# aliftffd/ViT-vs-Raw-IQ

Measured on AMD Instinct MI355X. Metric: IQ frames/sec training (fwd+loss+bwd+clip+AdamW), higher is better.
Workload: dtype bf16; 1 GPU; ViT-Tiny/16 224x224 C=1 19cls (BASELINE configs[1]); config_id=B, per_gpu_batch=256, global_batch=256, parallelism=dp1, hipgraph=True

## Files before the change

### vit-vs-raw-iq_amd/csrc/attention.hip

```cpp
#include <stdlib.h>

#include "common.h"
#include "iqvit.h"
#include "prof.h"

namespace {

constexpr int ATT_THREADS = 512;
constexpr int ATT_WAVES = ATT_THREADS / 64;
constexpr float LOG2E = 1.4426950408889634f;
constexpr float LN2 = 0.6931471805599453f;
constexpr float NEG_BIG = -1.0e30f;

__device__ __forceinline__ float fast_exp2(float x) { return __builtin_amdgcn_exp2f(x); }

template <int DH> struct AttCfg {
  static constexpr int LD = (DH == 16) ? 16 : DH + 16;
  static constexpr int KS = (DH + 31) / 32;
  static constexpr int DT = DH / 16;
  static constexpr int CPR = DH / 8;
};

typedef __attribute__((address_space(3))) s16x4 lds_s16x4;

__device__ __forceinline__ bf16x8 tr_frag(const bf16* tile, int ld, int r0, int c0, int lane) {
  const int i16 = lane & 15, g = lane >> 4;
  const bf16* a = tile + (r0 + 4 * g + (i16 >> 2)) * ld + c0 + 4 * (i16 & 3);
  s16x4 lo = __builtin_amdgcn_ds_read_tr16_b64_v4i16((lds_s16x4*)(a));
  s16x4 hi = __builtin_amdgcn_ds_read_tr16_b64_v4i16((lds_s16x4*)(a + 16 * ld));
  s16x8 v = {lo[0], lo[1], lo[2], lo[3], hi[0], hi[1], hi[2], hi[3]};
  return __builtin_bit_cast(bf16x8, v);
}

template <int DH>
__device__ __forceinline__ bf16x8 row_frag_lds(const bf16* tile, int row, int s, int lane) {
  const int d0 = s * 32 + 8 * (lane >> 4);
  bf16x8 v = {};
  if (DH >= 32 || d0 < DH) v = *reinterpret_cast<const bf16x8*>(tile + row * AttCfg<DH>::LD + d0);
  return v;
}
template <int DH>
__device__ __forceinline__ bf16x8 row_frag_gmem(const bf16* base, long ldg, int row, int nrows, int s, int lane) {
  const int d0 = s * 32 + 8 * (lane >> 4);
  bf16x8 v = {};
  if (row < nrows && (DH >= 32 || d0 < DH)) v = *reinterpret_cast<const bf16x8*>(base + (long)row * ldg + d0);
  return v;
}

template <int DH>
__device__ __forceinline__ void stage_rows(bf16* img, const bf16* base, long ldg, int r_begin, int nrows_pad, int S,
                                           int tid) {
  constexpr int CPR = AttCfg<DH>::CPR, LD = AttCfg<DH>::LD;
  for (int id = tid; id < nrows_pad * CPR; id += ATT_THREADS) {
    const int r = id / CPR, c = id % CPR;
    bf16x8 v = {};
    if (r_begin + r < S) v = *reinterpret_cast<const bf16x8*>(base + (long)(r_begin + r) * ldg + c * 8);
    *reinterpret_cast<bf16x8*>(img + r * LD + c * 8) = v;
  }
}

template <int DH, int UN>
__device__ __forceinline__ void stage_pair(bf16* imgA, const bf16* baseA, long ldgA, bf16* imgB, const bf16* baseB, long ldgB,
                                           int r_begin, int nrows_pad, int S, int tid) {
  constexpr int CPR = AttCfg<DH>::CPR, LD = AttCfg<DH>::LD;
  const int total = nrows_pad * CPR;
  for (int base = 0; base < total; base += UN * ATT_THREADS) {
    bf16x8 va[UN], vb[UN];
#pragma unroll
    for (int j = 0; j < UN; ++j) {
      const int id = min(base + j * ATT_THREADS + tid, total - 1);
      const int r = min(r_begin + id / CPR, S - 1), c = id % CPR;
      va[j] = *reinterpret_cast<const bf16x8*>(baseA + (long)r * ldgA + c * 8);
      vb[j] = *reinterpret_cast<const bf16x8*>(baseB + (long)r * ldgB + c * 8);
    }
#pragma unroll
    for (int j = 0; j < UN; ++j) {
      const int id = base + j * ATT_THREADS + tid;
      const int r = id / CPR, c = id % CPR;
      if (id < total) {
        const bool live = r_begin + r < S;
        *reinterpret_cast<bf16x8*>(imgA + r * LD + c * 8) = live ? va[j] : bf16x8{};
        *reinterpret_cast<bf16x8*>(imgB + r * LD + c * 8) = live ? vb[j] : bf16x8{};
      }
    }
  }
}

__device__ __forceinline__ bf16x8 pack_b(const f32x4& lo, const f32x4& hi) {
  bf16x8 v;
#pragma unroll
  for (int r = 0; r < 4; ++r) { v[r] = (bf16)lo[r]; v[4 + r] = (bf16)hi[r]; }
  return v;
}

__device__ __forceinline__ float group4_max(float v) {
  v = fmaxf(v, __shfl_xor(v, 16, 64));
  return fmaxf(v, __shfl_xor(v, 32, 64));
}
__device__ __forceinline__ float group4_sum(float v) {
  v += __shfl_xor(v, 16, 64);
  return v + __shfl_xor(v, 32, 64);
}

template <int DH, bool MASKED>
__global__ __launch_bounds__(ATT_THREADS) void attn_fwd_kernel(const bf16* __restrict__ qkv, bf16* __restrict__ out,
                                                               float* __restrict__ lse, const uint8_t* __restrict__ mask,
                                                               long mask_hstride, int S, int H, int kchunk,
                                                               float scale_log2, float masked_raw) {
  using C = AttCfg<DH>;
  extern __shared__ __attribute__((aligned(16))) unsigned char smem[];
  bf16* Ks = reinterpret_cast<bf16*>(smem);
  bf16* Vs = Ks + kchunk * C::LD;
  const int tid = threadIdx.x, lane = tid & 63, wave = tid >> 6, g = lane >> 4, c16 = lane & 15;
  const int b = blockIdx.x / H, h = blockIdx.x % H;
  const int D = H * DH;
  const long ldg = 3L * D;
  const bf16* qb = qkv + (long)b * S * ldg + h * DH;
  const bf16* kb_ = qb + D;
  const bf16* vb_ = qb + 2 * D;
  const uint8_t* mk = MASKED ? mask + (long)b * (mask_hstride ? (long)H * S * S : (long)S * S) + h * mask_hstride : nullptr;
  const int qtiles = (S + 31) / 32, npass = (qtiles + ATT_WAVES - 1) / ATT_WAVES, nstage = (S + kchunk - 1) / kchunk;

  if (nstage == 1) {
    stage_pair<DH, 4>(Ks, kb_, ldg, Vs, vb_, ldg, 0, min(kchunk, ((S + 31) / 32) * 32), S, tid);
    __syncthreads();
  }
  for (int pass = 0; pass < npass; ++pass) {
    const int qt = pass * ATT_WAVES + wave;
    const bool active = qt < qtiles;
    bf16x8 qf[2][C::KS];
    f32x4 o[2][C::DT];
    float m[2], lsum[2];
#pragma unroll
    for (int u = 0; u < 2; ++u) {
      m[u] = NEG_BIG; lsum[u] = 0.f;
#pragma unroll
      for (int s = 0; s < C::KS; ++s) qf[u][s] = row_frag_gmem<DH>(qb, ldg, qt * 32 + u * 16 + c16, active ? S : 0, s, lane);
#pragma unroll
      for (int dt = 0; dt < C::DT; ++dt) o[u][dt] = f32x4{0.f, 0.f, 0.f, 0.f};
    }
    for (int st = 0; st < nstage; ++st) {
      const int k0 = st * kchunk;
      const int krows = min(kchunk, ((S - k0 + 31) / 32) * 32);
      if (nstage > 1) {
        __syncthreads();
        stage_pair<DH, 2>(Ks, kb_, ldg, Vs, vb_, ldg, k0, krows, S, tid);
        __syncthreads();
      }
      if (active) {
        const bool u1 = qt * 32 + 16 < S;
        for (int kb = 0; kb < krows; kb += 32) {
          const bool k1 = k0 + kb + 16 < S;
          const bool kpad = k0 + kb + 32 > S;
          f32x4 sc[2][2];
#pragma unroll
          for (int kt = 0; kt < 2; ++kt) {
            if (kt == 1 && !k1) {
              sc[0][1] = f32x4{0.f, 0.f, 0.f, 0.f}; sc[1][1] = f32x4{0.f, 0.f, 0.f, 0.f};
              continue;
            }
            bf16x8 kf[C::KS];
#pragma unroll
            for (int s = 0; s < C::KS; ++s) kf[s] = row_frag_lds<DH>(Ks, kb + kt * 16 + c16, s, lane);
#pragma unroll
            for (int u = 0; u < 2; ++u) {
              f32x4 a = {0.f, 0.f, 0.f, 0.f};
              if (u == 0 || u1) {
#pragma unroll
                for (int s = 0; s < C::KS; ++s) a = __builtin_amdgcn_mfma_f32_16x16x32_bf16(kf[s], qf[u][s], a, 0, 0, 0);
              }
              sc[u][kt] = a;
            }
          }
          bf16x8 pb[2];
#pragma unroll
          for (int u = 0; u < 2; ++u) {
            if (u == 1 && !u1) { pb[1] = bf16x8{}; continue; }
            float mx = NEG_BIG;
#pragma unroll
            for (int kt = 0; kt < 2; ++kt) {
              if (kt == 1 && !k1) continue;
#pragma unroll
              for (int r = 0; r < 4; ++r) {
                float x = sc[u][kt][r];
                if (MASKED) {
                  const int key = k0 + kb + kt * 16 + 4 * g + r;
                  const int q = qt * 32 + u * 16 + c16;
                  if (key < S && q < S && !mk[(long)q * S + key]) x = masked_raw;
                }
                if (kpad) {
                  const int key = k0 + kb + kt * 16 + 4 * g + r;
                  x = key < S ? x : NEG_BIG;
                }
                sc[u][kt][r] = x;
                mx = fmaxf(mx, x);
              }
            }
            mx = group4_max(mx) * scale_log2;
            const float mn = fmaxf(m[u], mx);
            const float alpha = fast_exp2(m[u] - mn);
            m[u] = mn;
            float rs = 0.f;
#pragma unroll
            for (int kt = 0; kt < 2; ++kt) {
              if (kt == 1 && !k1) continue;
#pragma unroll
              for (int r = 0; r < 4; ++r) {
                const float pv = fast_exp2(fmaf(sc[u][kt][r], scale_log2, -mn));
                sc[u][kt][r] = pv;
                rs += pv;
              }
            }
            lsum[u] = lsum[u] * alpha + rs;
#pragma unroll
            for (int dt = 0; dt < C::DT; ++dt) o[u][dt] *= alpha;
            pb[u] = pack_b(sc[u][0], sc[u][1]);
          }
#pragma unroll
          for (int dt = 0; dt < C::DT; ++dt) {
            const bf16x8 vt = tr_frag(Vs, C::LD, kb, dt * 16, lane);
            o[0][dt] = __builtin_amdgcn_mfma_f32_16x16x32_bf16(vt, pb[0], o[0][dt], 0, 0, 0);
            if (u1) o[1][dt] = __builtin_amdgcn_mfma_f32_16x16x32_bf16(vt, pb[1], o[1][dt], 0, 0, 0);
          }
        }
      }
    }
    if (active) {
#pragma unroll
      for (int u = 0; u < 2; ++u) {
        const float l = group4_sum(lsum[u]);
        const float inv = 1.0f / l;
        const int q = qt * 32 + u * 16 + c16;
        if (q < S) {
#pragma unroll
          for (int dt = 0; dt < C::DT; ++dt) {
            bf16x4 w;
#pragma unroll
            for (int r = 0; r < 4; ++r) w[r] = (bf16)(o[u][dt][r] * inv);
            *reinterpret_cast<bf16x4*>(out + ((long)b * S + q) * D + h * DH + dt * 16 + 4 * g) = w;
          }
          if (g == 0) lse[((long)b * H + h) * S + q] = (m[u] + log2f(l)) * LN2;
        }
      }
    }
  }
}

template <int DH, bool MASKED>
__global__ __launch_bounds__(ATT_THREADS, 4) void attn_bwd_kernel(const bf16* __restrict__ qkv, const bf16* __restrict__ out,
                                                               const bf16* __restrict__ dout, const float* __restrict__ lse,
                                                               bf16* __restrict__ dqkv, const uint8_t* __restrict__ mask,
                                                               long mask_hstride, int S, int H, int spad, int chunk,
                                                               float scale, float masked_raw) {
  using C = AttCfg<DH>;
  extern __shared__ __attribute__((aligned(16))) unsigned char smem[];
  bf16* I0 = reinterpret_cast<bf16*>(smem);
  bf16* I1 = I0 + chunk * C::LD;
  float* lse_s = reinterpret_cast<float*>(I1 + chunk * C::LD);
  float* del_s = lse_s + spad;
  const int tid = threadIdx.x, lane = tid & 63, wave = tid >> 6, g = lane >> 4, c16 = lane & 15;
  const int b = blockIdx.x / H, h = blockIdx.x % H;
  const int D = H * DH;
  const long ldg = 3L * D;
  const bf16* qb = qkv + (long)b * S * ldg + h * DH;
  const bf16* kb_ = qb + D;
  const bf16* vb_ = qb + 2 * D;
  const bf16* ob = out + (long)b * S * D + h * DH;
  const bf16* dob = dout + (long)b * S * D + h * DH;
  bf16* dqb = dqkv + (long)b * S * ldg + h * DH;
  const uint8_t* mk = MASKED ? mask + (long)b * (mask_hstride ? (long)H * S * S : (long)S * S) + h * mask_hstride : nullptr;
  const float scale_log2 = scale * LOG2E;
  const int nblk = spad / 32;
  const int nchunk = (spad + chunk - 1) / chunk;
  const bool single = nchunk == 1;

  if (single) {
    stage_pair<DH, 4>(I0, qb, ldg, I1, dob, (long)D, 0, spad, S, tid);
    __syncthreads();
  }
  for (int q = tid; q < spad; q += ATT_THREADS) {
    float dl = 0.f, ls = 0.f;
    if (q < S) {
#pragma unroll
      for (int c = 0; c < C::CPR; ++c) {
        const bf16x8 a = single ? *reinterpret_cast<const bf16x8*>(I1 + q * C::LD + c * 8)
                                : *reinterpret_cast<const bf16x8*>(dob + (long)q * D + c * 8);
        const bf16x8 o8 = *reinterpret_cast<const bf16x8*>(ob + (long)q * D + c * 8);
#pragma unroll
        for (int e = 0; e < 8; ++e) dl += (float)a[e] * (float)o8[e];
      }
      ls = lse[((long)b * H + h) * S + q] * LOG2E;
    }
    del_s[q] = dl;
    lse_s[q] = ls;
  }
  __syncthreads();

  const int nunit = (S + 15) / 16;
  for (int ug = 0; ug * ATT_WAVES < nunit; ++ug) {
    const int unit = ug * ATT_WAVES + wave;
    const bool have = unit < nunit;
    bf16x8 kf[C::KS], vf[C::KS];
#pragma unroll
    for (int s = 0; s < C::KS; ++s) {
      kf[s] = row_frag_gmem<DH>(kb_, ldg, unit * 16 + c16, have ? S : 0, s, lane);
      vf[s] = row_frag_gmem<DH>(vb_, ldg, unit * 16 + c16, have ? S : 0, s, lane);
    }
    f32x4 dv[C::DT], dk[C::DT];
#pragma unroll
    for (int dt = 0; dt < C::DT; ++dt) { dv[dt] = f32x4{0.f, 0.f, 0.f, 0.f}; dk[dt] = f32x4{0.f, 0.f, 0.f, 0.f}; }
    const int key = unit * 16 + c16;
    const bool unit_partial = unit * 16 + 16 > S;
    for (int qc = 0; qc < nchunk; ++qc) {
      const int q0 = qc * chunk;
      const int rows = min(chunk, spad - q0);
      if (!single) {
        __syncthreads();
        stage_pair<DH, 2>(I0, qb, ldg, I1, dob, (long)D, q0, rows, S, tid);
        __syncthreads();
      }
      if (!have) continue;
      for (int ql = 0; ql < rows; ql += 32) {
        const bool u1 = q0 + ql + 16 < S;
        f32x4 p[2], ds[2];
#pragma unroll
        for (int u = 0; u < 2; ++u) {
          if (u == 1 && !u1) { p[1] = f32x4{0.f, 0.f, 0.f, 0.f}; ds[1] = f32x4{0.f, 0.f, 0.f, 0.f}; continue; }
          f32x4 sa = {0.f, 0.f, 0.f, 0.f}, dp = {0.f, 0.f, 0.f, 0.f};
#pragma unroll
          for (int s = 0; s < C::KS; ++s) {
            const bf16x8 qa = row_frag_lds<DH>(I0, ql + u * 16 + c16, s, lane);
            const bf16x8 da = row_frag_lds<DH>(I1, ql + u * 16 + c16, s, lane);
            sa = __builtin_amdgcn_mfma_f32_16x16x32_bf16(qa, kf[s], sa, 0, 0, 0);
            dp = __builtin_amdgcn_mfma_f32_16x16x32_bf16(da, vf[s], dp, 0, 0, 0);
          }
#pragma unroll
          for (int r = 0; r < 4; ++r) {
            const int q = q0 + ql + u * 16 + 4 * g + r;
            bool blocked = false;
            if (MASKED) blocked = q < S && key < S && !mk[(long)q * S + key];
            float pv = fast_exp2((blocked ? masked_raw : sa[r]) * scale_log2 - lse_s[q]);
            if (unit_partial) pv = key < S ? pv : 0.f;
            p[u][r] = pv;
            ds[u][r] = blocked ? 0.f : pv * (dp[r] - del_s[q]) * scale;
          }
        }
        const bf16x8 pB = pack_b(p[0], p[1]), dsB = pack_b(ds[0], ds[1]);
#pragma unroll
        for (int dt = 0; dt < C::DT; ++dt) {
          const bf16x8 doT = tr_frag(I1, C::LD, ql, dt * 16, lane);
          const bf16x8 qT = tr_frag(I0, C::LD, ql, dt * 16, lane);
          dv[dt] = __builtin_amdgcn_mfma_f32_16x16x32_bf16(doT, pB, dv[dt], 0, 0, 0);
          dk[dt] = __builtin_amdgcn_mfma_f32_16x16x32_bf16(qT, dsB, dk[dt], 0, 0, 0);
        }
      }
    }
    if (have && key < S) {
#pragma unroll
      for (int dt = 0; dt < C::DT; ++dt) {
        bf16x4 wk, wv;
#pragma unroll
        for (int r = 0; r < 4; ++r) { wk[r] = (bf16)dk[dt][r]; wv[r] = (bf16)dv[dt][r]; }
        *reinterpret_cast<bf16x4*>(dqb + (long)key * ldg + D + dt * 16 + 4 * g) = wk;
        *reinterpret_cast<bf16x4*>(dqb + (long)key * ldg + 2 * D + dt * 16 + 4 * g) = wv;
      }
    }
  }

  bf16x8 qf[2][C::KS], dof[2][C::KS];
  if (single) {
#pragma unroll
    for (int u = 0; u < 2; ++u)
#pragma unroll
      for (int s = 0; s < C::KS; ++s) {
        const int q = min(wave, nblk - 1) * 32 + u * 16 + c16;
        qf[u][s] = row_frag_lds<DH>(I0, q, s, lane);
        dof[u][s] = row_frag_lds<DH>(I1, q, s, lane);
      }
  }
  for (int qg = 0; qg * ATT_WAVES < nblk; ++qg) {
    const int qblk = qg * ATT_WAVES + wave;
    const bool have = qblk < nblk;
    float lq[2], dl[2];
#pragma unroll
    for (int u = 0; u < 2; ++u) {
      const int q = min(qblk, nblk - 1) * 32 + u * 16 + c16;
      if (!single || qg != 0) {
#pragma unroll
        for (int s = 0; s < C::KS; ++s) {
          qf[u][s] = row_frag_gmem<DH>(qb, ldg, q, have ? S : 0, s, lane);
          dof[u][s] = row_frag_gmem<DH>(dob, (long)D, q, have ? S : 0, s, lane);
        }
      }
      lq[u] = lse_s[q];
      dl[u] = del_s[q];
    }
    f32x4 dq[C::DT][2];
#pragma unroll
    for (int dt = 0; dt < C::DT; ++dt)
#pragma unroll
      for (int u = 0; u < 2; ++u) dq[dt][u] = f32x4{0.f, 0.f, 0.f, 0.f};
    for (int kc = 0; kc < nchunk; ++kc) {
      const int k0 = kc * chunk;
      const int rows = min(chunk, spad - k0);
      if (!single || qg == 0) {
        __syncthreads();
        stage_pair<DH, 2>(I0, kb_, ldg, I1, vb_, ldg, k0, rows, S, tid);
        __syncthreads();
      }
      if (!have) continue;
      const bool u1 = qblk * 32 + 16 < S;
      for (int kl = 0; kl < rows; kl += 32) {
        const bool kblk_partial = k0 + kl + 32 > S;
        const bool k1 = k0 + kl + 16 < S;
        f32x4 ds[2][2];
#pragma unroll
        for (int kt = 0; kt < 2; ++kt) {
          if (kt == 1 && !k1) { ds[0][1] = f32x4{0.f, 0.f, 0.f, 0.f}; ds[1][1] = f32x4{0.f, 0.f, 0.f, 0.f}; continue; }
          bf16x8 ka[C::KS], va[C::KS];
#pragma unroll
          for (int s = 0; s < C::KS; ++s) {
            ka[s] = row_frag_lds<DH>(I0, kl + kt * 16 + c16, s, lane);
            va[s] = row_frag_lds<DH>(I1, kl + kt * 16 + c16, s, lane);
          }
#pragma unroll
          for (int u = 0; u < 2; ++u) {
            if (u == 1 && !u1) { ds[1][kt] = f32x4{0.f, 0.f, 0.f, 0.f}; continue; }
            f32x4 sa = {0.f, 0.f, 0.f, 0.f}, dp = {0.f, 0.f, 0.f, 0.f};
#pragma unroll
            for (int s = 0; s < C::KS; ++s) {
              sa = __builtin_amdgcn_mfma_f32_16x16x32_bf16(ka[s], qf[u][s], sa, 0, 0, 0);
              dp = __builtin_amdgcn_mfma_f32_16x16x32_bf16(va[s], dof[u][s], dp, 0, 0, 0);
            }
#pragma unroll
            for (int r = 0; r < 4; ++r) {
              const int key = k0 + kl + kt * 16 + 4 * g + r;
              bool blocked = false;
              if (MASKED) {
                const int q = qblk * 32 + u * 16 + c16;
                blocked = q < S && key < S && !mk[(long)q * S + key];
              }
              float pv = fast_exp2((blocked ? masked_raw : sa[r]) * scale_log2 - lq[u]);
              if (kblk_partial) pv = key < S ? pv : 0.f;
              ds[u][kt][r] = blocked ? 0.f : pv * (dp[r] - dl[u]) * scale;
            }
          }
        }
        bf16x8 dsB[2];
#pragma unroll
        for (int u = 0; u < 2; ++u) dsB[u] = pack_b(ds[u][0], ds[u][1]);
#pragma unroll
        for (int dt = 0; dt < C::DT; ++dt) {
          const bf16x8 kT = tr_frag(I0, C::LD, kl, dt * 16, lane);
          dq[dt][0] = __builtin_amdgcn_mfma_f32_16x16x32_bf16(kT, dsB[0], dq[dt][0], 0, 0, 0);
          if (u1) dq[dt][1] = __builtin_amdgcn_mfma_f32_16x16x32_bf16(kT, dsB[1], dq[dt][1], 0, 0, 0);
        }
      }
    }
    if (have) {
#pragma unroll
      for (int u = 0; u < 2; ++u) {
        const int q = qblk * 32 + u * 16 + c16;
        if (q < S) {
#pragma unroll
          for (int dt = 0; dt < C::DT; ++dt) {
            bf16x4 w;
#pragma unroll
            for (int r = 0; r < 4; ++r) w[r] = (bf16)dq[dt][u][r];
            *reinterpret_cast<bf16x4*>(dqb + (long)q * ldg + dt * 16 + 4 * g) = w;
          }
        }
      }
    }
  }
}

template <int DH>
__device__ __forceinline__ bf16x8 row_frag_img(const bf16* tile, int ld, int row, int s, int lane) {
  const int d0 = s * 32 + 8 * (lane >> 4);
  bf16x8 v = {};
  if (DH >= 32 || d0 < DH) v = *reinterpret_cast<const bf16x8*>(tile + row * ld + d0);
  return v;
}

template <int UN>
__device__ __forceinline__ void stage_block(bf16* img, int ld, const bf16* src, int cols, int S, int spad, int tid, int nthr) {
  const int cpr = cols >> 3, total = spad * cpr, live = S * cpr;
  for (int base = 0; base < total; base += UN * nthr) {
    bf16x8 v[UN];
#pragma unroll
    for (int j = 0; j < UN; ++j) {
      const int id = min(base + j * nthr + tid, live - 1);
      v[j] = *reinterpret_cast<const bf16x8*>(src + (long)id * 8);
    }
#pragma unroll
    for (int j = 0; j < UN; ++j) {
      const int id = base + j * nthr + tid;
      if (id < total) {
        const int r = id / cpr, c = id - r * cpr;
        *reinterpret_cast<bf16x8*>(img + r * ld + c * 8) = id < live ? v[j] : bf16x8{};
      }
    }
  }
}

template <int DH, int G>
__global__ __launch_bounds__(ATT_THREADS) void attn_frame_fwd_kernel(const bf16* __restrict__ qkv, bf16* __restrict__ out,
                                                                     float* __restrict__ lse, int S, int H, int spad,
                                                                     float scale_log2) {
  using C = AttCfg<DH>;
  extern __shared__ __attribute__((aligned(16))) unsigned char smem[];
  bf16* img = reinterpret_cast<bf16*>(smem);
  const int tid = threadIdx.x, lane = tid & 63, wave = tid >> 6, g = lane >> 4, c16 = lane & 15;
  const int nwave = blockDim.x >> 6;
  const int b = blockIdx.x;
  const int D = H * DH, ld = 3 * D + 16;
  stage_block<8>(img, ld, qkv + (long)b * S * 3 * D, 3 * D, S, spad, tid, blockDim.x);
  __syncthreads();
  const int qtiles = (S + 31) / 32;
  for (int h = wave; h < H; h += nwave) {
    const bf16* Qs = img + h * DH;
    const bf16* Ks = Qs + D;
    const bf16* Vs = Qs + 2 * D;
    for (int qt0 = 0; qt0 < qtiles; qt0 += G) {
      bf16x8 qf[G][2][C::KS];
      f32x4 o[G][2][C::DT];
      float m[G][2], lsum[G][2];
      bool live[G][2];
#pragma unroll
      for (int t = 0; t < G; ++t)
#pragma unroll
        for (int u = 0; u < 2; ++u) {
          const int q0 = (qt0 + t) * 32 + u * 16;
          live[t][u] = q0 < S;
          m[t][u] = NEG_BIG; lsum[t][u] = 0.f;
#pragma unroll
          for (int s = 0; s < C::KS; ++s) qf[t][u][s] = row_frag_img<DH>(Qs, ld, min(q0 + c16, spad - 1), s, lane);
#pragma unroll
          for (int dt = 0; dt < C::DT; ++dt) o[t][u][dt] = f32x4{0.f, 0.f, 0.f, 0.f};
        }
      for (int kb = 0; kb < spad; kb += 32) {
        const bool k1 = kb + 16 < S;
        bf16x8 kf[2][C::KS], vt[C::DT];
#pragma unroll
        for (int kt = 0; kt < 2; ++kt)
#pragma unroll
          for (int s = 0; s < C::KS; ++s) kf[kt][s] = row_frag_img<DH>(Ks, ld, kb + kt * 16 + c16, s, lane);
#pragma unroll
        for (int dt = 0; dt < C::DT; ++dt) vt[dt] = tr_frag(Vs, ld, kb, dt * 16, lane);
#pragma unroll
        for (int t = 0; t < G; ++t)
#pragma unroll
          for (int u = 0; u < 2; ++u) {
            if (!live[t][u]) continue;
            f32x4 sc[2];
#pragma unroll
            for (int kt = 0; kt < 2; ++kt) {
              f32x4 a = {0.f, 0.f, 0.f, 0.f};
              if (kt == 0 || k1) {
#pragma unroll
                for (int s = 0; s < C::KS; ++s) a = __builtin_amdgcn_mfma_f32_16x16x32_bf16(kf[kt][s], qf[t][u][s], a, 0, 0, 0);
              }
              sc[kt] = a;
            }
            float mx = NEG_BIG;
#pragma unroll
            for (int kt = 0; kt < 2; ++kt) {
              if (kt == 1 && !k1) { sc[1] = f32x4{0.f, 0.f, 0.f, 0.f}; continue; }
#pragma unroll
              for (int r = 0; r < 4; ++r) {
                const int key = kb + kt * 16 + 4 * g + r;
                const float x = key < S ? sc[kt][r] : NEG_BIG;
                sc[kt][r] = x;
                mx = fmaxf(mx, x);
              }
            }
            mx = group4_max(mx) * scale_log2;
            const float mn = fmaxf(m[t][u], mx);
            const float alpha = fast_exp2(m[t][u] - mn);
            m[t][u] = mn;
            float rs = 0.f;
#pragma unroll
            for (int kt = 0; kt < 2; ++kt) {
              if (kt == 1 && !k1) continue;
#pragma unroll
              for (int r = 0; r < 4; ++r) {
                const float pv = fast_exp2(fmaf(sc[kt][r], scale_log2, -mn));
                sc[kt][r] = pv;
                rs += pv;
              }
            }
            lsum[t][u] = lsum[t][u] * alpha + rs;
            const bf16x8 pb = pack_b(sc[0], sc[1]);
#pragma unroll
            for (int dt = 0; dt < C::DT; ++dt) {
              o[t][u][dt] *= alpha;
              o[t][u][dt] = __builtin_amdgcn_mfma_f32_16x16x32_bf16(vt[dt], pb, o[t][u][dt], 0, 0, 0);
            }
          }
      }
#pragma unroll
      for (int t = 0; t < G; ++t)
#pragma unroll
        for (int u = 0; u < 2; ++u) {
          if (!live[t][u]) continue;
          const float l = group4_sum(lsum[t][u]);
          const float inv = 1.0f / l;
          const int q = (qt0 + t) * 32 + u * 16 + c16;
          if (q < S) {
#pragma unroll
            for (int dt = 0; dt < C::DT; ++dt) {
              bf16x4 w;
#pragma unroll
              for (int r = 0; r < 4; ++r) w[r] = (bf16)(o[t][u][dt][r] * inv);
              *reinterpret_cast<bf16x4*>(out + ((long)b * S + q) * D + h * DH + dt * 16 + 4 * g) = w;
            }
            if (g == 0) lse[((long)b * H + h) * S + q] = (m[t][u] + log2f(l)) * LN2;
          }
        }
    }
  }
}

template <int DH, int UG, int QG>
__global__ __launch_bounds__(ATT_THREADS) void attn_frame_bwd_kernel(const bf16* __restrict__ qkv, const bf16* __restrict__ out,
                                                                     const bf16* __restrict__ dout, const float* __restrict__ lse,
                                                                     bf16* __restrict__ dqkv, int S, int H, int spad, float scale) {
  using C = AttCfg<DH>;
  extern __shared__ __attribute__((aligned(16))) unsigned char smem[];
  const int tid = threadIdx.x, lane = tid & 63, wave = tid >> 6, g = lane >> 4, c16 = lane & 15;
  const int nwave = blockDim.x >> 6;
  const int b = blockIdx.x;
  const int D = H * DH, ld = 3 * D + 16, ldo = D + 16;
  bf16* img = reinterpret_cast<bf16*>(smem);
  bf16* dimg = img + spad * ld;
  float* lse_s = reinterpret_cast<float*>(dimg + spad * ldo);
  float* del_s = lse_s + H * spad;
  const long ldg = 3L * D;
  const float scale_log2 = scale * LOG2E;
  for (int id = tid; id < spad * H; id += blockDim.x) {
    const int q = id / H, h = id - q * H;
    float dl = 0.f, ls = 0.f;
    if (q < S) {
      const bf16* orow = out + ((long)b * S + q) * D + h * DH;
      const bf16* drow = dout + ((long)b * S + q) * D + h * DH;
#pragma unroll
      for (int c = 0; c < C::CPR; ++c) {
        const bf16x8 a = *reinterpret_cast<const bf16x8*>(drow + c * 8);
        const bf16x8 o8 = *reinterpret_cast<const bf16x8*>(orow + c * 8);
#pragma unroll
        for (int e = 0; e < 8; ++e) dl += (float)a[e] * (float)o8[e];
      }
      ls = lse[((long)b * H + h) * S + q] * LOG2E;
    }
    del_s[h * spad + q] = dl;
    lse_s[h * spad + q] = ls;
  }
  stage_block<8>(img, ld, qkv + (long)b * S * ldg, 3 * D, S, spad, tid, blockDim.x);
  stage_block<4>(dimg, ldo, dout + (long)b * S * D, D, S, spad, tid, blockDim.x);
  __syncthreads();
  bf16* dqb = dqkv + (long)b * S * ldg;
  const int nunit = (S + 15) / 16, nblk = spad / 32;
  for (int h = wave; h < H; h += nwave) {
    const bf16* Qs = img + h * DH;
    const bf16* Ks = Qs + D;
    const bf16* Vs = Qs + 2 * D;
    const bf16* Os = dimg + h * DH;
    const float* lq_s = lse_s + h * spad;
    const float* dl_s = del_s + h * spad;
    for (int un0 = 0; un0 < nunit; un0 += UG) {
      bf16x8 kf[UG][C::KS], vf[UG][C::KS];
      f32x4 dv[UG][C::DT], dk[UG][C::DT];
#pragma unroll
      for (int j = 0; j < UG; ++j) {
        const int row = min((un0 + j) * 16 + c16, spad - 1);
#pragma unroll
        for (int s = 0; s < C::KS; ++s) {
          kf[j][s] = row_frag_img<DH>(Ks, ld, row, s, lane);
          vf[j][s] = row_frag_img<DH>(Vs, ld, row, s, lane);
        }
#pragma unroll
        for (int dt = 0; dt < C::DT; ++dt) { dv[j][dt] = f32x4{0.f, 0.f, 0.f, 0.f}; dk[j][dt] = f32x4{0.f, 0.f, 0.f, 0.f}; }
      }
      for (int ql = 0; ql < spad; ql += 32) {
        const bool u1 = ql + 16 < S;
        bf16x8 qa[2][C::KS], da[2][C::KS], doT[C::DT], qT[C::DT];
        f32x4 lq4[2], dl4[2];
#pragma unroll
        for (int u = 0; u < 2; ++u) {
#pragma unroll
          for (int s = 0; s < C::KS; ++s) {
            qa[u][s] = row_frag_img<DH>(Qs, ld, ql + u * 16 + c16, s, lane);
            da[u][s] = row_frag_img<DH>(Os, ldo, ql + u * 16 + c16, s, lane);
          }
          lq4[u] = *reinterpret_cast<const f32x4*>(lq_s + ql + u * 16 + 4 * g);
          dl4[u] = *reinterpret_cast<const f32x4*>(dl_s + ql + u * 16 + 4 * g);
        }
#pragma unroll
        for (int dt = 0; dt < C::DT; ++dt) {
          doT[dt] = tr_frag(Os, ldo, ql, dt * 16, lane);
          qT[dt] = tr_frag(Qs, ld, ql, dt * 16, lane);
        }
#pragma unroll
        for (int j = 0; j < UG; ++j) {
          const int unit = un0 + j;
          if (unit >= nunit) continue;
          const int key = unit * 16 + c16;
          const bool unit_partial = unit * 16 + 16 > S;
          f32x4 p[2], ds[2];
#pragma unroll
          for (int u = 0; u < 2; ++u) {
            if (u == 1 && !u1) { p[1] = f32x4{0.f, 0.f, 0.f, 0.f}; ds[1] = f32x4{0.f, 0.f, 0.f, 0.f}; continue; }
            f32x4 sa = {0.f, 0.f, 0.f, 0.f}, dp = {0.f, 0.f, 0.f, 0.f};
#pragma unroll
            for (int s = 0; s < C::KS; ++s) {
              sa = __builtin_amdgcn_mfma_f32_16x16x32_bf16(qa[u][s], kf[j][s], sa, 0, 0, 0);
              dp = __builtin_amdgcn_mfma_f32_16x16x32_bf16(da[u][s], vf[j][s], dp, 0, 0, 0);
            }
#pragma unroll
            for (int r = 0; r < 4; ++r) {
              float pv = fast_exp2(sa[r] * scale_log2 - lq4[u][r]);
              if (unit_partial) pv = key < S ? pv : 0.f;
              p[u][r] = pv;
              ds[u][r] = pv * (dp[r] - dl4[u][r]) * scale;
            }
          }
          const bf16x8 pB = pack_b(p[0], p[1]), dsB = pack_b(ds[0], ds[1]);
#pragma unroll
          for (int dt = 0; dt < C::DT; ++dt) {
            dv[j][dt] = __builtin_amdgcn_mfma_f32_16x16x32_bf16(doT[dt], pB, dv[j][dt], 0, 0, 0);
            dk[j][dt] = __builtin_amdgcn_mfma_f32_16x16x32_bf16(qT[dt], dsB, dk[j][dt], 0, 0, 0);
          }
        }
      }
#pragma unroll
      for (int j = 0; j < UG; ++j) {
        const int key = (un0 + j) * 16 + c16;
        if (un0 + j < nunit && key < S) {
#pragma unroll
          for (int dt = 0; dt < C::DT; ++dt) {
            bf16x4 wk, wv;
#pragma unroll
            for (int r = 0; r < 4; ++r) { wk[r] = (bf16)dk[j][dt][r]; wv[r] = (bf16)dv[j][dt][r]; }
            *reinterpret_cast<bf16x4*>(dqb + (long)key * ldg + D + h * DH + dt * 16 + 4 * g) = wk;
            *reinterpret_cast<bf16x4*>(dqb + (long)key * ldg + 2 * D + h * DH + dt * 16 + 4 * g) = wv;
          }
        }
      }
    }
    for (int qb0 = 0; qb0 < nblk; qb0 += QG) {
      bf16x8 qf[QG][2][C::KS], dof[QG][2][C::KS];
      float lq[QG][2], dl[QG][2];
      bool live[QG][2];
      f32x4 dq[QG][C::DT][2];
#pragma unroll
      for (int t = 0; t < QG; ++t)
#pragma unroll
        for (int u = 0; u < 2; ++u) {
          const int q0 = (qb0 + t) * 32 + u * 16;
          live[t][u] = q0 < S;
          const int q = min(q0 + c16, spad - 1);
#pragma unroll
          for (int s = 0; s < C::KS; ++s) {
            qf[t][u][s] = row_frag_img<DH>(Qs, ld, q, s, lane);
            dof[t][u][s] = row_frag_img<DH>(Os, ldo, q, s, lane);
          }
          lq[t][u] = lq_s[q];
          dl[t][u] = dl_s[q];
#pragma unroll
          for (int dt = 0; dt < C::DT; ++dt) dq[t][dt][u] = f32x4{0.f, 0.f, 0.f, 0.f};
        }
      for (int kl = 0; kl < spad; kl += 32) {
        const bool kblk_partial = kl + 32 > S;
        const bool k1 = kl + 16 < S;
        bf16x8 ka[2][C::KS], va[2][C::KS], kT[C::DT];
#pragma unroll
        for (int kt = 0; kt < 2; ++kt)
#pragma unroll
          for (int s = 0; s < C::KS; ++s) {
            ka[kt][s] = row_frag_img<DH>(Ks, ld, kl + kt * 16 + c16, s, lane);
            va[kt][s] = row_frag_img<DH>(Vs, ld, kl + kt * 16 + c16, s, lane);
          }
#pragma unroll
        for (int dt = 0; dt < C::DT; ++dt) kT[dt] = tr_frag(Ks, ld, kl, dt * 16, lane);
#pragma unroll
        for (int t = 0; t < QG; ++t)
#pragma unroll
          for (int u = 0; u < 2; ++u) {
            if (!live[t][u]) continue;
            f32x4 ds[2];
#pragma unroll
            for (int kt = 0; kt < 2; ++kt) {
              if (kt == 1 && !k1) { ds[1] = f32x4{0.f, 0.f, 0.f, 0.f}; continue; }
              f32x4 sa = {0.f, 0.f, 0.f, 0.f}, dp = {0.f, 0.f, 0.f, 0.f};
#pragma unroll
              for (int s = 0; s < C::KS; ++s) {
                sa = __builtin_amdgcn_mfma_f32_16x16x32_bf16(ka[kt][s], qf[t][u][s], sa, 0, 0, 0);
                dp = __builtin_amdgcn_mfma_f32_16x16x32_bf16(va[kt][s], dof[t][u][s], dp, 0, 0, 0);
              }
#pragma unroll
              for (int r = 0; r < 4; ++r) {
                const int key = kl + kt * 16 + 4 * g + r;
                float pv = fast_exp2(sa[r] * scale_log2 - lq[t][u]);
                if (kblk_partial) pv = key < S ? pv : 0.f;
                ds[kt][r] = pv * (dp[r] - dl[t][u]) * scale;
              }
            }
            const bf16x8 dsB = pack_b(ds[0], ds[1]);
#pragma unroll
            for (int dt = 0; dt < C::DT; ++dt)
              dq[t][dt][u] = __builtin_amdgcn_mfma_f32_16x16x32_bf16(kT[dt], dsB, dq[t][dt][u], 0, 0, 0);
          }
      }
#pragma unroll
      for (int t = 0; t < QG; ++t)
#pragma unroll
        for (int u = 0; u < 2; ++u) {
          const int q = (qb0 + t) * 32 + u * 16 + c16;
          if (live[t][u] && q < S) {
#pragma unroll
            for (int dt = 0; dt < C::DT; ++dt) {
              bf16x4 w;
#pragma unroll
              for (int r = 0; r < 4; ++r) w[r] = (bf16)dq[t][dt][u][r];
              *reinterpret_cast<bf16x4*>(dqb + (long)q * ldg + h * DH + dt * 16 + 4 * g) = w;
            }
          }
        }
    }
  }
}

constexpr size_t ATT_FRAME_LDS_MAX = 112 * 1024;
inline size_t frame_fwd_lds(int S, int H, int dh) {
  const int spad = (S + 31) / 32 * 32;
  return (size_t)spad * (3 * H * dh + 16) * 2;
}
inline size_t frame_bwd_lds(int S, int H, int dh) {
  const int spad = (S + 31) / 32 * 32;
  return (size_t)spad * (3 * H * dh + 16) * 2 + (size_t)spad * (H * dh + 16) * 2 + (size_t)2 * H * spad * sizeof(float);
}
inline bool use_frame(int S, size_t lds) {
  static const int tune = [] { const char* e = getenv("IQ_TUNE_ATTN_FRAME"); return e ? atoi(e) : -1; }();
  if (lds > ATT_FRAME_LDS_MAX) return false;
  if (tune == 0) return false;
  if (tune == 1) return true;
  return S <= 128;
}

template <int DH>
int launch_frame_fwd(const void* qkv, void* out, float* lse, int B, int S, int H, hipStream_t st) {
  const int spad = (S + 31) / 32 * 32;
  const size_t lds = frame_fwd_lds(S, H, DH);
  auto k = attn_frame_fwd_kernel<DH, (DH == 64 ? 2 : 4)>;
  if (lds > 48 * 1024) (void)hipFuncSetAttribute((const void*)k, hipFuncAttributeMaxDynamicSharedMemorySize, (int)lds);
  const int threads = 64 * (H < ATT_WAVES ? H : ATT_WAVES);
  k<<<B, threads, lds, st>>>((const bf16*)qkv, (bf16*)out, lse, S, H, spad, LOG2E / sqrtf((float)DH));
  return iq_launch_status();
}
template <int DH>
int launch_frame_bwd(const void* qkv, const void* out, const void* dout, const float* lse, void* dqkv, int B, int S, int H,
                     hipStream_t st) {
  const int spad = (S + 31) / 32 * 32;
  const size_t lds = frame_bwd_lds(S, H, DH);
  auto k = attn_frame_bwd_kernel<DH, (DH == 64 ? 2 : 3), (DH == 16 ? 4 : DH == 32 ? 3 : 2)>;
  if (lds > 48 * 1024) (void)hipFuncSetAttribute((const void*)k, hipFuncAttributeMaxDynamicSharedMemorySize, (int)lds);
  const int threads = 64 * (H < ATT_WAVES ? H : ATT_WAVES);
  k<<<B, threads, lds, st>>>((const bf16*)qkv, (const bf16*)out, (const bf16*)dout, lse, (bf16*)dqkv, S, H, spad,
                             1.0f / sqrtf((float)DH));
  return iq_launch_status();
}

constexpr size_t ATT_LDS_FWD_BUDGET = 72 * 1024;
constexpr size_t ATT_LDS_BWD_BUDGET = 76 * 1024;
constexpr int ATT_MAX_S = 4096;

template <int DH> int bwd_chunk_rows(int S) {
  const int spad = (S + 31) / 32 * 32;
  const long room = (long)ATT_LDS_BWD_BUDGET - (long)2 * spad * sizeof(float);
  int chunk = (int)(room / (2 * AttCfg<DH>::LD * 2)) / 32 * 32;
  if (chunk > spad) chunk = spad;
  return chunk;
}
template <int DH> size_t bwd_lds_bytes(int S) {
  const int spad = (S + 31) / 32 * 32;
  return (size_t)2 * bwd_chunk_rows<DH>(S) * AttCfg<DH>::LD * 2 + (size_t)2 * spad * sizeof(float);
}

template <int DH, bool MASKED>
int launch_fwd(const void* qkv, void* out, float* lse, const uint8_t* mask, long mask_hstride, int B, int S, int H,
               hipStream_t st) {
  const int spad = (S + 31) / 32 * 32;
  int kchunk = (int)(ATT_LDS_FWD_BUDGET / (2 * AttCfg<DH>::LD * 2)) / 32 * 32;
  if (kchunk > spad) kchunk = spad;
  const size_t lds = (size_t)2 * kchunk * AttCfg<DH>::LD * 2;
  const float scale_log2 = LOG2E / sqrtf((float)DH);
  if (lds > 48 * 1024)
    (void)hipFuncSetAttribute((const void*)attn_fwd_kernel<DH, MASKED>, hipFuncAttributeMaxDynamicSharedMemorySize, (int)lds);
  attn_fwd_kernel<DH, MASKED><<<B * H, ATT_THREADS, lds, st>>>((const bf16*)qkv, (bf16*)out, lse, mask, mask_hstride, S, H,
                                                               kchunk, scale_log2, -10000.0f * sqrtf((float)DH));
  return iq_launch_status();
}

template <int DH, bool MASKED>
int launch_bwd(const void* qkv, const void* out, const void* dout, const float* lse, void* dqkv, const uint8_t* mask,
               long mask_hstride, int B, int S, int H, hipStream_t st) {
  const int spad = (S + 31) / 32 * 32;
  const int chunk = bwd_chunk_rows<DH>(S);
  if (S > ATT_MAX_S || chunk < 32) return IQ_ERR_UNSUPPORTED;
  const size_t lds = bwd_lds_bytes<DH>(S);
  if (lds > 48 * 1024)
    (void)hipFuncSetAttribute((const void*)attn_bwd_kernel<DH, MASKED>, hipFuncAttributeMaxDynamicSharedMemorySize, (int)lds);
  attn_bwd_kernel<DH, MASKED><<<B * H, ATT_THREADS, lds, st>>>((const bf16*)qkv, (const bf16*)out, (const bf16*)dout, lse,
                                                               (bf16*)dqkv, mask, mask_hstride, S, H, spad, chunk,
                                                               1.0f / sqrtf((float)DH), -10000.0f * sqrtf((float)DH));
  return iq_launch_status();
}

template <bool MASKED>
int dispatch_fwd(const void* qkv, void* out, float* lse, const uint8_t* mask, long hs, int B, int S, int H, int dh,
                 hipStream_t st) {
  switch (dh) {
    case 16: return launch_fwd<16, MASKED>(qkv, out, lse, mask, hs, B, S, H, st);
    case 32: return launch_fwd<32, MASKED>(qkv, out, lse, mask, hs, B, S, H, st);
    case 64: return launch_fwd<64, MASKED>(qkv, out, lse, mask, hs, B, S, H, st);
    default: return IQ_ERR_UNSUPPORTED;
  }
}
template <bool MASKED>
int dispatch_bwd(const void* qkv, const void* out, const void* dout, const float* lse, void* dqkv, const uint8_t* mask,
                 long hs, int B, int S, int H, int dh, hipStream_t st) {
  switch (dh) {
    case 16: return launch_bwd<16, MASKED>(qkv, out, dout, lse, dqkv, mask, hs, B, S, H, st);
    case 32: return launch_bwd<32, MASKED>(qkv, out, dout, lse, dqkv, mask, hs, B, S, H, st);
    case 64: return launch_bwd<64, MASKED>(qkv, out, dout, lse, dqkv, mask, hs, B, S, H, st);
    default: return IQ_ERR_UNSUPPORTED;
  }
}

}

extern "C" int iq_attn_supported(int S, int dh) {
  if (S <= 0 || S > ATT_MAX_S) return 0;
  return (dh == 16 || dh == 32 || dh == 64) ? 1 : 0;
}

extern "C" int iq_attn_fwd_masked(const void* qkv, void* out, float* lse, const uint8_t* mask, long mask_hstride, int B,
                                  int S, int H, int dh, iq_stream_t stream) {
  if (B <= 0) return IQ_OK;
  if (!qkv || !out || !lse || S <= 0 || H <= 0) return IQ_ERR_ARG;
  if (mask_hstride != 0 && mask_hstride != (long)S * S) return IQ_ERR_ARG;
  hipStream_t st = (hipStream_t)stream;
  IQ_PROF(IQ_FAM_ATTN_FWD, st);
  const bool frame = !mask && (dh == 16 || dh == 32 || dh == 64) && use_frame(S, frame_fwd_lds(S, H, dh));
  {
    const double rows = (double)B * S, Dm = (double)H * dh;
    if (frame) IQ_PROF_K(2.0 * rows * 4.0 * Dm + 4.0 * B * H * S, 4.0 * B * H * (double)S * S * dh, "attn_frame_fwd_kernel<%d>", dh);
    else IQ_PROF_K(2.0 * rows * 4.0 * Dm + 4.0 * B * H * S, 4.0 * B * H * (double)S * S * dh, "attn_fwd_kernel<%d, %s>", dh, mask ? "true" : "false");
  }
  if (frame) {
    switch (dh) {
      case 16: return launch_frame_fwd<16>(qkv, out, lse, B, S, H, st);
      case 32: return launch_frame_fwd<32>(qkv, out, lse, B, S, H, st);
      default: return launch_frame_fwd<64>(qkv, out, lse, B, S, H, st);
    }
  }
  return mask ? dispatch_fwd<true>(qkv, out, lse, mask, mask_hstride, B, S, H, dh, st)
              : dispatch_fwd<false>(qkv, out, lse, nullptr, 0, B, S, H, dh, st);
}
extern "C" int iq_attn_fwd(const void* qkv, void* out, float* lse, int B, int S, int H, int dh, iq_stream_t stream) {
  return iq_attn_fwd_masked(qkv, out, lse, nullptr, 0, B, S, H, dh, stream);
}

extern "C" int iq_attn_bwd_masked(const void* qkv, const void* out, const void* dout, const float* lse, void* dqkv,
                                  const uint8_t* mask, long mask_hstride, int B, int S, int H, int dh,
                                  iq_stream_t stream) {
  if (B <= 0) return IQ_OK;
  if (!qkv || !out || !dout || !lse || !dqkv || S <= 0 || H <= 0) return IQ_ERR_ARG;
  if (mask_hstride != 0 && mask_hstride != (long)S * S) return IQ_ERR_ARG;
  hipStream_t st = (hipStream_t)stream;
  IQ_PROF(IQ_FAM_ATTN_BWD, st);
  const bool frame = !mask && (dh == 16 || dh == 32 || dh == 64) && use_frame(S, frame_bwd_lds(S, H, dh));
  {
    const double rows = (double)B * S, Dm = (double)H * dh;
    if (frame) IQ_PROF_K(2.0 * rows * 8.0 * Dm + 4.0 * B * H * S, 14.0 * B * H * (double)S * S * dh, "attn_frame_bwd_kernel<%d>", dh);
    else IQ_PROF_K(2.0 * rows * 8.0 * Dm + 4.0 * B * H * S, 14.0 * B * H * (double)S * S * dh, "attn_bwd_kernel<%d, %s>", dh, mask ? "true" : "false");
  }
  if (frame) {
    switch (dh) {
      case 16: return launch_frame_bwd<16>(qkv, out, dout, lse, dqkv, B, S, H, st);
      case 32: return launch_frame_bwd<32>(qkv, out, dout, lse, dqkv, B, S, H, st);
      default: return launch_frame_bwd<64>(qkv, out, dout, lse, dqkv, B, S, H, st);
    }
  }
  return mask ? dispatch_bwd<true>(qkv, out, dout, lse, dqkv, mask, mask_hstride, B, S, H, dh, st)
              : dispatch_bwd<false>(qkv, out, dout, lse, dqkv, nullptr, 0, B, S, H, dh, st);
}
extern "C" int iq_attn_bwd(const void* qkv, const void* out, const void* dout, const float* lse, void* dqkv, int B,
                           int S, int H, int dh, iq_stream_t stream) {
  return iq_attn_bwd_masked(qkv, out, dout, lse, dqkv, nullptr, 0, B, S, H, dh, stream);
}
```

Measured before the change: 51240 frames/s.

## Add single-pass attention backward kernel that keeps dS in LDS for dh=64

Adds a new attention backward kernel for unmasked dh=64 with short sequences (padded length up to 224). It stages Q and dO in swizzled LDS and computes P and dS once per key block, accumulating dK and dV. It writes dS into an LDS matrix, then restages K and computes dQ from the stored dS, so the score matrix is not recomputed. The cost is a large LDS footprint, roughly one workgroup per CU, plus a 1024-thread block. The path is selected when the frame kernel is not used, and an environment variable can tune or disable it.

```diff
diff --git a/vit-vs-raw-iq_amd/csrc/attention.hip b/vit-vs-raw-iq_amd/csrc/attention.hip
--- a/vit-vs-raw-iq_amd/csrc/attention.hip
+++ b/vit-vs-raw-iq_amd/csrc/attention.hip
@@ -475,6 +475,200 @@
   }
 }
 
+constexpr int ONCE_MAX_SPAD = 224;
+constexpr int ONCE_LD = 64;
+
+__device__ __forceinline__ int once_off(int row, int col) { return row * ONCE_LD + (col ^ (((row >> 1) & 3) << 4)); }
+
+__device__ __forceinline__ bf16x8 once_tr_frag(const bf16* tile, int r0, int dt, int lane) {
+  const int i16 = lane & 15, g = lane >> 4;
+  const bf16* a = tile + once_off(r0 + 4 * g + (i16 >> 2), dt * 16 + 4 * (i16 & 3));
+  s16x4 lo = __builtin_amdgcn_ds_read_tr16_b64_v4i16((lds_s16x4*)(a));
+  s16x4 hi = __builtin_amdgcn_ds_read_tr16_b64_v4i16((lds_s16x4*)(a + 16 * ONCE_LD));
+  s16x8 v = {lo[0], lo[1], lo[2], lo[3], hi[0], hi[1], hi[2], hi[3]};
+  return __builtin_bit_cast(bf16x8, v);
+}
+__device__ __forceinline__ bf16x8 once_row_frag(const bf16* tile, int row, int s, int lane) {
+  return *reinterpret_cast<const bf16x8*>(tile + once_off(row, s * 32 + 8 * (lane >> 4)));
+}
+
+template <int NT, int UN, int NIMG>
+__device__ __forceinline__ void once_stage(bf16* const (&img)[NIMG], const bf16* const (&base)[NIMG],
+                                           const long (&ldg)[NIMG], int spad, int S, int tid) {
+  const int total = spad * 8;
+  for (int b0 = 0; b0 < total; b0 += UN * NT) {
+    bf16x8 v[NIMG][UN];
+#pragma unroll
+    for (int j = 0; j < UN; ++j) {
+      const int id = min(b0 + j * NT + tid, total - 1);
+      const int r = min(id >> 3, S - 1), c = id & 7;
+#pragma unroll
+      for (int i = 0; i < NIMG; ++i) v[i][j] = *reinterpret_cast<const bf16x8*>(base[i] + (long)r * ldg[i] + c * 8);
+    }
+#pragma unroll
+    for (int j = 0; j < UN; ++j) {
+      const int id = b0 + j * NT + tid;
+      const int r = id >> 3, c = id & 7;
+      if (id < total) {
+        const bool live = r < S;
+#pragma unroll
+        for (int i = 0; i < NIMG; ++i) *reinterpret_cast<bf16x8*>(img[i] + once_off(r, c * 8)) = live ? v[i][j] : bf16x8{};
+      }
+    }
+  }
+}
+
+template <int NT>
+__global__ __launch_bounds__(NT, 4) void attn_bwd_once_kernel(const bf16* __restrict__ qkv, const bf16* __restrict__ out,
+                                                              const bf16* __restrict__ dout, const float* __restrict__ lse,
+                                                              bf16* __restrict__ dqkv, int S, int H, int spad, float scale) {
+  constexpr int DH = 64, KS = 2, DT = 4, NW = NT / 64;
+  extern __shared__ __attribute__((aligned(16))) unsigned char smem[];
+  bf16* I0 = reinterpret_cast<bf16*>(smem);
+  bf16* I1 = I0 + spad * ONCE_LD;
+  float* lse_s = reinterpret_cast<float*>(I1 + spad * ONCE_LD);
+  float* del_s = lse_s + spad;
+  bf16* dSi = reinterpret_cast<bf16*>(del_s + spad);
+  const int tid = threadIdx.x, lane = tid & 63, wave = tid >> 6, g = lane >> 4, c16 = lane & 15;
+  const int b = blockIdx.x / H, h = blockIdx.x % H;
+  const int D = H * DH;
+  const long ldg = 3L * D;
+  const bf16* qb = qkv + (long)b * S * ldg + h * DH;
+  const bf16* kb_ = qb + D;
+  const bf16* vb_ = qb + 2 * D;
+  const bf16* ob = out + (long)b * S * D + h * DH;
+  const bf16* dob = dout + (long)b * S * D + h * DH;
+  bf16* dqb = dqkv + (long)b * S * ldg + h * DH;
+  const float scale_log2 = scale * LOG2E;
+  const int nunit = (S + 15) / 16;
+  const int ldS = nunit * 16 + 8;
+
+  {
+    bf16* const img[2] = {I0, I1};
+    const bf16* const src[2] = {qb, dob};
+    const long lds_[2] = {ldg, (long)D};
+    once_stage<NT, 2048 / NT, 2>(img, src, lds_, spad, S, tid);
+  }
+  __syncthreads();
+  for (int q = tid; q < spad; q += NT) {
+    float dl = 0.f, ls = 0.f;
+    if (q < S) {
+#pragma unroll
+      for (int c = 0; c < 8; ++c) {
+        const bf16x8 a = *reinterpret_cast<const bf16x8*>(I1 + once_off(q, c * 8));
+        const bf16x8 o8 = *reinterpret_cast<const bf16x8*>(ob + (long)q * D + c * 8);
+#pragma unroll
+        for (int e = 0; e < 8; ++e) dl += (float)a[e] * (float)o8[e];
+      }
+      ls = lse[((long)b * H + h) * S + q] * LOG2E;
+    }
+    del_s[q] = dl;
+    lse_s[q] = ls;
+  }
+  __syncthreads();
+
+  for (int unit = wave; unit < nunit; unit += NW) {
+    bf16x8 kf[KS], vf[KS];
+#pragma unroll
+    for (int s = 0; s < KS; ++s) {
+      kf[s] = row_frag_gmem<DH>(kb_, ldg, unit * 16 + c16, S, s, lane);
+      vf[s] = row_frag_gmem<DH>(vb_, ldg, unit * 16 + c16, S, s, lane);
+    }
+    f32x4 dv[DT], dk[DT];
+#pragma unroll
+    for (int dt = 0; dt < DT; ++dt) { dv[dt] = f32x4{0.f, 0.f, 0.f, 0.f}; dk[dt] = f32x4{0.f, 0.f, 0.f, 0.f}; }
+    const int key = unit * 16 + c16;
+    const bool unit_partial = unit * 16 + 16 > S;
+    for (int ql = 0; ql < spad; ql += 32) {
+      const bool u1 = ql + 16 < S;
+      f32x4 p[2], ds[2];
+#pragma unroll
+      for (int u = 0; u < 2; ++u) {
+        if (u == 1 && !u1) { p[1] = f32x4{0.f, 0.f, 0.f, 0.f}; ds[1] = f32x4{0.f, 0.f, 0.f, 0.f}; continue; }
+        f32x4 sa = {0.f, 0.f, 0.f, 0.f}, dp = {0.f, 0.f, 0.f, 0.f};
+#pragma unroll
+        for (int s = 0; s < KS; ++s) {
+          const bf16x8 qa = once_row_frag(I0, ql + u * 16 + c16, s, lane);
+          const bf16x8 da = once_row_frag(I1, ql + u * 16 + c16, s, lane);
+          sa = __builtin_amdgcn_mfma_f32_16x16x32_bf16(qa, kf[s], sa, 0, 0, 0);
+          dp = __builtin_amdgcn_mfma_f32_16x16x32_bf16(da, vf[s], dp, 0, 0, 0);
+        }
+        const f32x4 lq4 = *reinterpret_cast<const f32x4*>(lse_s + ql + u * 16 + 4 * g);
+        const f32x4 dl4 = *reinterpret_cast<const f32x4*>(del_s + ql + u * 16 + 4 * g);
+#pragma unroll
+        for (int r = 0; r < 4; ++r) {
+          float pv = fast_exp2(sa[r] * scale_log2 - lq4[r]);
+          if (unit_partial) pv = key < S ? pv : 0.f;
+          p[u][r] = pv;
+          ds[u][r] = pv * (dp[r] - dl4[r]) * scale;
+        }
+      }
+      const bf16x8 pB = pack_b(p[0], p[1]), dsB = pack_b(ds[0], ds[1]);
+      bf16* w = dSi + (ql + 4 * g) * ldS + key;
+#pragma unroll
+      for (int r = 0; r < 4; ++r) w[r * ldS] = dsB[r];
+      if (u1) {
+#pragma unroll
+        for (int r = 0; r < 4; ++r) w[(16 + r) * ldS] = dsB[4 + r];
+      }
+#pragma unroll
+      for (int dt = 0; dt < DT; ++dt) {
+        const bf16x8 doT = once_tr_frag(I1, ql, dt, lane);
+        const bf16x8 qT = once_tr_frag(I0, ql, dt, lane);
+        dv[dt] = __builtin_amdgcn_mfma_f32_16x16x32_bf16(doT, pB, dv[dt], 0, 0, 0);
+        dk[dt] = __builtin_amdgcn_mfma_f32_16x16x32_bf16(qT, dsB, dk[dt], 0, 0, 0);
+      }
+    }
+    if (key < S) {
+#pragma unroll
+      for (int dt = 0; dt < DT; ++dt) {
+        bf16x4 wk, wv;
+#pragma unroll
+        for (int r = 0; r < 4; ++r) { wk[r] = (bf16)dk[dt][r]; wv[r] = (bf16)dv[dt][r]; }
+        *reinterpret_cast<bf16x4*>(dqb + (long)key * ldg + D + dt * 16 + 4 * g) = wk;
+        *reinterpret_cast<bf16x4*>(dqb + (long)key * ldg + 2 * D + dt * 16 + 4 * g) = wv;
+      }
+    }
+  }
+
+  __syncthreads();
+  {
+    bf16* const img[1] = {I0};
+    const bf16* const src[1] = {kb_};
+    const long lds_[1] = {ldg};
+    once_stage<NT, 2048 / NT, 1>(img, src, lds_, spad, S, tid);
+  }
+  __syncthreads();
+  for (int half = wave; half < nunit; half += NW) {
+    const int q = half * 16 + c16;
+    const bf16* drow = dSi + q * ldS + 4 * g;
+    f32x4 dq[DT];
+#pragma unroll
+    for (int dt = 0; dt < DT; ++dt) dq[dt] = f32x4{0.f, 0.f, 0.f, 0.f};
+    for (int kl = 0; kl < spad; kl += 32) {
+      const bool k1 = kl + 16 < S;
+      const bf16x4 lo = *reinterpret_cast<const bf16x4*>(drow + kl);
+      bf16x4 hi = {};
+      if (k1) hi = *reinterpret_cast<const bf16x4*>(drow + kl + 16);
+      const bf16x8 dsB = {lo[0], lo[1], lo[2], lo[3], hi[0], hi[1], hi[2], hi[3]};
+#pragma unroll
+      for (int dt = 0; dt < DT; ++dt) {
+        const bf16x8 kT = once_tr_frag(I0, kl, dt, lane);
+        dq[dt] = __builtin_amdgcn_mfma_f32_16x16x32_bf16(kT, dsB, dq[dt], 0, 0, 0);
+      }
+    }
+    if (q < S) {
+#pragma unroll
+      for (int dt = 0; dt < DT; ++dt) {
+        bf16x4 w;
+#pragma unroll
+        for (int r = 0; r < 4; ++r) w[r] = (bf16)dq[dt][r];
+        *reinterpret_cast<bf16x4*>(dqb + (long)q * ldg + dt * 16 + 4 * g) = w;
+      }
+    }
+  }
+}
+
 template <int DH>
 __device__ __forceinline__ bf16x8 row_frag_img(const bf16* tile, int ld, int row, int s, int lane) {
   const int d0 = s * 32 + 8 * (lane >> 4);
@@ -917,6 +1111,23 @@
   return iq_launch_status();
 }
 
+inline int once_threads(int S, int dh, bool masked) {
+  static const int tune = [] { const char* e = getenv("IQ_TUNE_ATTN_BWD_ONCE"); return e ? atoi(e) : -1; }();
+  if (masked || dh != 64 || (S + 31) / 32 * 32 > ONCE_MAX_SPAD || tune == 0) return 0;
+  return tune == 512 ? 512 : 1024;
+}
+template <int NT>
+int launch_bwd_once(const void* qkv, const void* out, const void* dout, const float* lse, void* dqkv, int B, int S, int H,
+                    hipStream_t st) {
+  const int spad = (S + 31) / 32 * 32, nunit = (S + 15) / 16;
+  const size_t lds = (size_t)2 * spad * ONCE_LD * 2 + (size_t)2 * spad * sizeof(float) + (size_t)spad * (nunit * 16 + 8) * 2;
+  auto k = attn_bwd_once_kernel<NT>;
+  if (lds > 48 * 1024) (void)hipFuncSetAttribute((const void*)k, hipFuncAttributeMaxDynamicSharedMemorySize, (int)lds);
+  k<<<B * H, NT, lds, st>>>((const bf16*)qkv, (const bf16*)out, (const bf16*)dout, lse, (bf16*)dqkv, S, H, spad,
+                            1.0f / sqrtf(64.0f));
+  return iq_launch_status();
+}
+
 template <bool MASKED>
 int dispatch_fwd(const void* qkv, void* out, float* lse, const uint8_t* mask, long hs, int B, int S, int H, int dh,
                  hipStream_t st) {
@@ -981,9 +1192,11 @@
   hipStream_t st = (hipStream_t)stream;
   IQ_PROF(IQ_FAM_ATTN_BWD, st);
   const bool frame = !mask && (dh == 16 || dh == 32 || dh == 64) && use_frame(S, frame_bwd_lds(S, H, dh));
+  const int once = frame ? 0 : once_threads(S, dh, mask != nullptr);
   {
     const double rows = (double)B * S, Dm = (double)H * dh;
     if (frame) IQ_PROF_K(2.0 * rows * 8.0 * Dm + 4.0 * B * H * S, 14.0 * B * H * (double)S * S * dh, "attn_frame_bwd_kernel<%d>", dh);
+    else if (once) IQ_PROF_K(2.0 * rows * 8.0 * Dm + 4.0 * B * H * S, 10.0 * B * H * (double)S * S * dh, "attn_bwd_once_kernel<%d>", once);
     else IQ_PROF_K(2.0 * rows * 8.0 * Dm + 4.0 * B * H * S, 14.0 * B * H * (double)S * S * dh, "attn_bwd_kernel<%d, %s>", dh, mask ? "true" : "false");
   }
   if (frame) {
@@ -993,6 +1206,8 @@
       default: return launch_frame_bwd<64>(qkv, out, dout, lse, dqkv, B, S, H, st);
     }
   }
+  if (once == 512) return launch_bwd_once<512>(qkv, out, dout, lse, dqkv, B, S, H, st);
+  if (once) return launch_bwd_once<1024>(qkv, out, dout, lse, dqkv, B, S, H, st);
   return mask ? dispatch_bwd<true>(qkv, out, dout, lse, dqkv, mask, mask_hstride, B, S, H, dh, st)
               : dispatch_bwd<false>(qkv, out, dout, lse, dqkv, nullptr, 0, B, S, H, dh, st);
 }
```

After: 51860 frames/s, median of 6. 1.2% higher.
